# stanfordnlp/mac-network

Measured on AMD Instinct MI355X. Metric: questions/sec fwd+bwd (B=64,d=512,p=12,KB=14x14x1024) at 1/2/4/8 MI355X, higher is better.
Workload: dtype f32 (3xfp16-split emulation); 1 GPU

## Files before the change

mac-network_amd/csrc/macx_chain_h2.hip.h:

```cpp
#pragma once
#include <hip/hip_ext.h>
#include "macx_chain_api.hip.h"

namespace macx {


template <int CTRL>
__device__ __forceinline__ float dpp_mov_f(float v) {
  return __builtin_bit_cast(float, __builtin_amdgcn_update_dpp(0, __builtin_bit_cast(int, v), CTRL, 0xF, 0xF, false));
}
__device__ __forceinline__ float row16_sum(float v) {
  v += dpp_mov_f<0x128>(v);
  v += dpp_mov_f<0x124>(v);
  v += dpp_mov_f<0x122>(v);
  v += dpp_mov_f<0x121>(v);
  return v;
}

__device__ __forceinline__ float row8_sum(float v) {
  v += dpp_mov_f<0x141>(v);
  v += dpp_mov_f<0x1B>(v);
  v += dpp_mov_f<0xB1>(v);
  return v;
}

__device__ __forceinline__ float chain_tanh(float x) {
  const float a = fabsf(x), x2 = x * x;
  float r = 62.0f / 2835.0f;
  r = fmaf(r, x2, -17.0f / 315.0f);
  r = fmaf(r, x2, 2.0f / 15.0f);
  r = fmaf(r, x2, -1.0f / 3.0f);
  r = fmaf(r, x2, 1.0f);
  r *= x;
  const float e = __expf(2.0f * fminf(a, 20.0f));
  const float t = 1.0f - 2.0f * __frcp_rn(e + 1.0f);
  return a < 0.3f ? r : copysignf(t, x);
}
__device__ __forceinline__ float chain_act(int act, float x) {
  if (act == ACT_ELU) return x > 0.0f ? x : __expf(x) - 1.0f;
  if (act == ACT_TANH) return chain_tanh(x);
  return act_apply(act, x);
}

template <int D_, int R_ = 64>
struct ChainGeo {
  static constexpr int D = D_, R = R_, KG = D / 8, CB = D / 128, KS = D / 32;
  static constexpr int TM = 16;
  static constexpr int NWC = D >= 512 ? 8 : 4;
  static constexpr int NWR = 8 / NWC;
  static constexpr int CW = D / NWC;
  static constexpr int RPW = R / NWR;
  static constexpr int RT = RPW / TM;
  static constexpr int CT = CW / 16;
  static constexpr int NRG = R / 16;
  static constexpr int WPG = 8 / NRG;
  static constexpr int IT = KG / (4 * WPG);
  static constexpr int SB = R / 8;
  static_assert(R == 64 || ((R == 32 || R == 16) && NWR == 1), "short tiles: every wave holds all rows (d = 512)");
  static constexpr size_t P_BYTES = (size_t)4 * R * D;
  static constexpr int QS = 5;
  static constexpr int BITS_LD = KG + 4;
  static constexpr size_t LDS = P_BYTES + (size_t)R * (8 + 8 + 1 + 1) * 4 + (size_t)(2 + 1 + QS) * D * 4 + (size_t)R * BITS_LD;
  static_assert((R * BITS_LD) % 16 == 0, "LDS carve-outs stay 16-byte aligned");
  static_assert(D % 128 == 0 && D >= 128 && D <= 512, "one workgroup holds 64 rows x D as H2 planes in LDS");
};

template <int D_, int R_ = 64>
struct ChainCtx {
  using G = ChainGeo<D_, R_>;
// ... 264 lines not shown
  __device__ __forceinline__ float colred_sum(float v) const {
    return row16_sum(v);
  }
  __device__ __forceinline__ bool row_writer() const { return ah == 0; }
  __device__ __forceinline__ bool col_writer() const { return ar == 0; }

  __device__ __forceinline__ void rowmax(const f32x4 (&acc)[RT][CT]) const {
#pragma unroll
    for (int t = 0; t < RT; ++t) {
      float m = 0.f;
#pragma unroll
      for (int c = 0; c < CT; ++c)
#pragma unroll
        for (int q = 0; q < 4; ++q) m = fmaxf(m, fabsf(acc[t][c][q]));
      m = rowred_max(m);
      if (row_writer()) sMax[wave * R + arow(t)] = m;
    }
  }
  __device__ __forceinline__ void emit(const f32x4 (&acc)[RT][CT], bool to_p, const H2View& out) const {
    const size_t Rp = out.Rp();
    const size_t opb = out.plane_bytes();
#pragma unroll
    for (int t = 0; t < RT; ++t) {
      const int row = arow(t);
      const float s = h2_pow2(row_exponent_epi(row));
      const bool st = out.base && row < nvalid;
#pragma unroll
      for (int c = 0; c < CT; ++c) {
        const f32x4 xv = acc[t][c] * s;
        u32x2 hi, lo;
        hi[0] = pk_f16(xv[0], xv[1]);
        hi[1] = pk_f16(xv[2], xv[3]);
        const f32x2_t b0 = unpk_f16(hi[0]), b1 = unpk_f16(hi[1]);
        lo[0] = pk_f16(xv[0] - b0[0], xv[1] - b0[1]);
        lo[1] = pk_f16(xv[2] - b1[0], xv[3] - b1[1]);
        const int kg = akg(c);
        const int half = ahalf();
        if (to_p) {
          char* d = P + ((size_t)kg * R + row) * 16 + half;
          *reinterpret_cast<u32x2*>(d) = hi;
          *reinterpret_cast<u32x2*>(d + (size_t)KG * R * 16) = lo;
        }
        if (st) {
          char* g = out.base + ((size_t)kg * Rp + grow0 + row) * 16 + half;
          *reinterpret_cast<u32x2*>(g) = hi;
          *reinterpret_cast<u32x2*>(g + opb) = lo;
        }
      }
    }
  }
  __device__ __forceinline__ void colsum(const f32x4 (&acc)[RT][CT], float* part) const {
#pragma unroll
    for (int c = 0; c < CT; ++c) {
#pragma unroll
      for (int q = 0; q < 4; ++q) {
        float s = acc[0][c][q];
#pragma unroll
        for (int t = 1; t < RT; ++t) s += acc[t][c][q];
        s = colred_sum(s);
        if (col_writer()) {
          const int col = acol(c) + q;
          if (NWR == 1) part[col] = s;
          else sCol[wr * D + col] = s;
        }
      }
    }
  }
  __device__ __forceinline__ void colsum_finish(float* part) const {
    if (NWR == 2)
      for (int c = tid; c < D; c += 512) part[c] = sCol[c] + sCol[D + c];
  }
};


template <int D_, int KV = 0, int R_ = 64>
__global__ __launch_bounds__(512) void chain_fwd_kernel(const ChainFwdP p) {
  using C = ChainCtx<D_, R_>;
  constexpr int D = C::D, R = C::R, KG = C::KG, CT = C::CT, RT = C::RT, IT = C::IT;
  extern __shared__ __attribute__((aligned(16))) char lds[];
  C x;
  x.init(lds, p.M, p.N);
  const int M = p.M;

  auto stage0 = [&](uint32_t k1, uint32_t k2, uint8_t* bits1, uint8_t* bytes2, const H2View& KBd) __attribute__((always_inline)) {
    float v[IT][8];
    float m = 0.f;
    const bool drop1 = p.thr1 < (1u << 24), drop2 = p.thr2 < (1u << 24);
    const uint32_t key1 = run_key(k1, p.word), key2 = run_key(k2, p.word);
    const size_t Rp2 = (size_t)M + H2_PAD_ROWS;
#pragma unroll
    for (int j = 0; j < IT; ++j) {
      const int kg = x.ckg(j);
      const float* src = p.kb + min(x.cgrow, (size_t)M - 1) * D + kg * 8;
      const f32x4 a0 = *reinterpret_cast<const f32x4*>(src), a1 = *reinterpret_cast<const f32x4*>(src + 4);
#pragma unroll
      for (int q = 0; q < 4; ++q) { v[j][q] = x.cvalid ? a0[q] : 0.f; v[j][4 + q] = x.cvalid ? a1[q] : 0.f; }
    }
#pragma unroll
    for (int j = 0; j < IT; ++j) {
      const int kg = x.ckg(j);
      const uint32_t e0 = p.first + (uint32_t)(x.cgrow * (size_t)p.dlog + kg * 8);
      if (drop1) {
        uint32_t byte = 0;
#pragma unroll
        for (int q = 0; q < 8; q += 2) byte |= keep_pair(e0 + q, key1, p.thr1) << q;
#pragma unroll
        for (int q = 0; q < 8; ++q) v[j][q] = ((byte >> q) & 1u) ? v[j][q] * p.inv1 : 0.f;
        if (bits1 && x.cvalid) bits1[x.cgrow * KG + kg] = (uint8_t)byte;
      }
      if (drop2) {
        uint32_t byte = 0;
#pragma unroll
        for (int q = 0; q < 8; q += 2) byte |= keep_pair(e0 + q, key2, p.thr2) << q;
        x.sBits[x.crow * C::G::BITS_LD + kg] = (uint8_t)byte;
        if (bytes2 && x.cvalid) bytes2[(size_t)kg * Rp2 + x.cgrow] = (uint8_t)byte;
      }
#pragma unroll
      for (int q = 0; q < 8; ++q) m = fmaxf(m, fabsf(v[j][q]));
    }
    x.convert_finish(v, m, x.sE, KBd);
  };
  if constexpr (D == 512) {
#ifdef MACX_FILL_PROF
#define MACX_STAMP(cond, k) do { if ((cond) && p.pre.step == 5 && p.pre.fail && x.tid == 0) p.pre.fail[-31 + (k)] = (uint32_t)__builtin_readcyclecounter(); } while (0)
#else
#define MACX_STAMP(cond, k) do { } while (0)
#endif
    if ((int)blockIdx.x < p.pre.nfill) {
      const int f = blockIdx.x, nf = p.pre.nfill;
      MACX_STAMP(f == 0, 0);
      float (*red)[16][20] = reinterpret_cast<float (*)[16][20]>(lds);
      const int half = x.tid >> 8, tl = x.tid & 255;
      auto signal = [&](uint32_t* c0, uint32_t* c1) __attribute__((always_inline)) {
        asm volatile("s_waitcnt vmcnt(0)" ::: "memory");
        __syncthreads();
        if (x.tid == 0 && c0) signal_counter(c0);
        if (x.tid == 64 && c1) signal_counter(c1);
      };
      static_assert(C::G::P_BYTES >= sizeof(float) * 16 * 16 * 20, "the fillers' linear tiles stay inside P: sPart is free");
      uint32_t* sGave = reinterpret_cast<uint32_t*>(x.sPart);
      auto wait_tiles = [&](uint32_t* ca, uint32_t* cb, uint32_t v) __attribute__((always_inline)) {
        if (x.tid == 0) {
          bool ok = wait_counter<4>(ca, v, HANDOFF_BUDGET, p.pre.fail, p.pre.status, p.pre.step, HANDOFF_WRITE);
          if (ok && cb != ca) ok = wait_counter<4>(cb, v, HANDOFF_BUDGET, p.pre.fail, p.pre.status, p.pre.step, HANDOFF_WRITE);
          *sGave = ok ? 0u : 1u;
        }
        __syncthreads();
        return __builtin_amdgcn_readfirstlane(*sGave) != 0u;
      };
      const bool tail = p.pre.wlin.n_out != 0;
      if (tail) {
        const LinP& wl = p.pre.wlin;
        const int ntx = wl.n_out / 32, nun = ntx * ((wl.rows + 15) / 16);
#pragma unroll 1
        for (int u0 = 2 * f; u0 < nun; u0 += 2 * nf) {
          const int ua = u0, ub = min(u0 + 1, nun - 1), bya = ua / ntx, byb = ub / ntx;
          const int u = half ? ub : ua;
          small_linear_tile<1, false, true, false, 2>(wl, u % ntx, u / ntx, 0, red + 8 * half, tl, u0 + half < nun);
          signal(p.pre.gflag + bya, u0 + 1 < nun ? p.pre.gflag + byb : nullptr);
        }
      }
      MACX_STAMP(f == 0, 1);
      if (p.pre.ylin.n_out) {
        const LinP& yl = p.pre.ylin;
        const int ntx = yl.n_out / 32, nunits = ntx * ((yl.rows + 15) / 16);
        const uint32_t wtiles = (uint32_t)(p.pre.wlin.n_out / 32);
#pragma unroll 1
        for (int u0 = 2 * f; u0 < nunits; u0 += 2 * nf) {
          const int ua = u0, ub = min(u0 + 1, nunits - 1), bya = ua / ntx, byb = ub / ntx;
          const bool gave = tail && wait_tiles(p.pre.gflag + bya, p.pre.gflag + byb, wtiles);
          const int u = half ? ub : ua;
          small_linear_tile<1, false, true, true, 2>(yl, u % ntx, u / ntx, 0, red + 8 * half, tl, u0 + half < nunits, gave);
          __syncthreads();
        }
        signal(p.pre.yflag, nullptr);
      }
      MACX_STAMP(f == 0, 2);
      if (p.pre.KBd.base) {
        const int ntile = (M + R - 1) / R;
#pragma unroll 1
        for (int t = f; t < ntile; t += p.pre.nfill) {
          x.set_tile((size_t)t);
          stage0(p.pre.key1, p.pre.key2, p.pre.bits1, p.pre.bytes2, p.pre.KBd);
        }
      }
      MACX_STAMP(f == 0, 3);
      return;
    }
    x.set_tile((size_t)blockIdx.x - p.pre.nfill);
    MACX_STAMP((int)blockIdx.x == p.pre.nfill, 8);
  }
  if (p.mode == 0) {
    stage0(p.key1, p.key2, p.bits1, p.bytes2, p.KBd);
  } else if (p.mode == 2) {
    if (p.thr2 < (1u << 24)) {
      const size_t Rp2 = (size_t)M + H2_PAD_ROWS;
      const int r = x.tid & 63, k0 = x.tid >> 6;
      const size_t gr = min(x.grow0 + r, (size_t)M - 1);
      if (r < R) {
#pragma unroll
        for (int j = 0; j < KG / 8; ++j) x.sBits[r * C::G::BITS_LD + k0 + 8 * j] = p.bytes2[(size_t)(k0 + 8 * j) * Rp2 + gr];
      }
    }
    x.load_tile(p.KBd, x.sE);
  } else {
    x.load_tile(p.X, x.sE);
  }
  if (p.dbg & 1) return;

  f32x4 acc[RT][CT];
  auto bias_act = [&](auto act_c, const int* eTab, int eW, const float* bias) __attribute__((always_inline)) {
    constexpr int ACT = decltype(act_c)::value;
#pragma unroll
    for (int c = 0; c < CT; ++c) {
      const f32x4 bv = *reinterpret_cast<const f32x4*>(bias + x.acol(c));
#pragma unroll
      for (int t = 0; t < RT; ++t) {
        const float s = h2_unscale(eTab[x.arow(t)], eW);
#pragma unroll
        for (int q = 0; q < 4; ++q) acc[t][c][q] = chain_act(ACT, fmaf(acc[t][c][q], s, bv[q]));
      }
    }
  };
  auto bias_act_any = [&](int act, const int* eTab, int eW, const float* bias) __attribute__((always_inline)) {
    switch (act) {
      case ACT_TANH: bias_act(std::integral_constant<int, ACT_TANH>{}, eTab, eW, bias); break;
      case ACT_SIGMOID: bias_act(std::integral_constant<int, ACT_SIGMOID>{}, eTab, eW, bias); break;
      case ACT_ELU: bias_act(std::integral_constant<int, ACT_ELU>{}, eTab, eW, bias); break;
      case ACT_RELU: bias_act(std::integral_constant<int, ACT_RELU>{}, eTab, eW, bias); break;
      default: bias_act(std::integral_constant<int, ACT_NON>{}, eTab, eW, bias); break;
    }
  };

  if (p.mode != 1) {
    x.zero_acc(acc);
    x.template kloop<KV>(acc, p.Wx.planes);
    bias_act(std::integral_constant<int, ACT_NON>{}, x.sE, *p.Wx.exp, p.bx);
    x.rowmax(acc);
    __syncthreads();
    x.emit(acc, true, p.X);
    x.publish_rows(x.sE, C::PASS_EPI, p.X);
    __syncthreads();
  }
  if (p.dbg & 2) return;

  x.zero_acc(acc);
  x.template kloop<KV>(acc, p.W1b.planes);
  constexpr bool YCOH = D == 512;
  if constexpr (YCOH) {
    MACX_STAMP((int)blockIdx.x == p.pre.nfill, 9);
    if (p.pre.ylin.n_out && x.tid == 0)
      *reinterpret_cast<uint32_t*>(x.sPart) =
          wait_counter<8>(p.pre.yflag, (uint32_t)p.pre.nfill, HANDOFF_BUDGET, p.pre.fail, p.pre.status, p.pre.step, HANDOFF_Y) ? 0u : 1u;
  }
  if constexpr (YCOH) MACX_STAMP((int)blockIdx.x == p.pre.nfill, 10);
  __syncthreads();
  bool ygave = false;
  if constexpr (YCOH) {
    if (p.pre.ylin.n_out) ygave = __builtin_amdgcn_readfirstlane(*reinterpret_cast<const uint32_t*>(x.sPart)) != 0u;
  }
  {
    float v[IT][8];
    float m = 0.f;
    const float inv = h2_pow2(-x.sE[x.crow]);
    const float* yq = p.y + x.qrow(x.cgrow) * D;
    auto ldy = [&](const float* q) __attribute__((always_inline)) {
      if constexpr (YCOH) {
        const uint64_t* q8 = reinterpret_cast<const uint64_t*>(q);
        const uint64_t lo = __hip_atomic_load(q8, __ATOMIC_RELAXED, __HIP_MEMORY_SCOPE_AGENT);
        const uint64_t hi = __hip_atomic_load(q8 + 1, __ATOMIC_RELAXED, __HIP_MEMORY_SCOPE_AGENT);
        return f32x4{__uint_as_float((uint32_t)lo), __uint_as_float((uint32_t)(lo >> 32)), __uint_as_float((uint32_t)hi),
                     __uint_as_float((uint32_t)(hi >> 32))};
      } else {
        return *reinterpret_cast<const f32x4*>(q);
      }
    };
#pragma unroll
    for (int j = 0; j < IT; ++j) {
      const int kg = x.ckg(j);
      const char* s = x.P + ((size_t)kg * R + x.crow) * 16;
      const u32x4 hi = *reinterpret_cast<const u32x4*>(s), lo = *reinterpret_cast<const u32x4*>(s + (size_t)KG * R * 16);
      float xv[8];
      h2_join8(hi, lo, inv, xv);
      const f32x4 y0 = ldy(yq + kg * 8), y1 = ldy(yq + kg * 8 + 4);
#pragma unroll
      for (int q = 0; q < 8; ++q) {
        v[j][q] = xv[q] * (q < 4 ? y0[q & 3] : y1[q & 3]);
        m = fmaxf(m, fabsf(v[j][q]));
      }
    }
    if (ygave) {
#pragma unroll
      for (int j = 0; j < IT; ++j)
#pragma unroll
        for (int q = 0; q < 8; ++q) v[j][q] = handoff_poison();
    }
    x.convert_finish(v, m, x.sE2, H2View{nullptr, M, D});
  }
  {
    const int de = *p.W1a.exp - *p.W1b.exp;
#pragma unroll
    for (int t = 0; t < RT; ++t) {
      const int k = x.sE2[x.arow(t)] - x.sE[x.arow(t)] + de;
#pragma unroll
      for (int c = 0; c < CT; ++c)
#pragma unroll
        for (int q = 0; q < 4; ++q) acc[t][c][q] = ldexpf(acc[t][c][q], k);
    }
  }
  x.template kloop<KV>(acc, p.W1a.planes);
  bias_act_any(p.act1, x.sE2, *p.W1a.exp, p.b1);
  x.rowmax(acc);
  __syncthreads();
  x.emit(acc, true, p.H1);
  x.publish_rows(x.sE, C::PASS_EPI, p.H1);
  __syncthreads();
  if (p.dbg & 4) return;

  x.zero_acc(acc);
  x.template kloop<KV>(acc, p.W2.planes);
  bias_act(std::integral_constant<int, ACT_NON>{}, x.sE, *p.W2.exp, p.b2);
  x.rowmax(acc);
  {
    const bool drop2 = p.thr2 < (1u << 24);
    auto logit_pass = [&](auto act_c) __attribute__((always_inline)) {
      constexpr int ACT = decltype(act_c)::value;
#pragma unroll
      for (int t = 0; t < RT; ++t) {
        const size_t gr = min(x.grow0 + x.arow(t), (size_t)M - 1);
        const float* cq = p.c + (size_t)((uint32_t)gr / (uint32_t)p.N) * D;
        float part = 0.f;
#pragma unroll
        for (int c = 0; c < CT; ++c) {
          const int col = x.acol(c);
          const f32x4 cv = *reinterpret_cast<const f32x4*>(cq + col);
          const f32x4 wv = *reinterpret_cast<const f32x4*>(p.wk + col);
          const uint32_t kb = drop2 ? (uint32_t)x.sBits[x.arow(t) * C::G::BITS_LD + (col >> 3)] >> (col & 4) : 0xFu;
#pragma unroll
          for (int q = 0; q < 4; ++q) {
            float g = chain_act(ACT, acc[t][c][q] * cv[q]);
            if (drop2) g = ((kb >> q) & 1u) ? g * p.inv2 : 0.f;
            part = fmaf(g, wv[q], part);
          }
        }
        part = x.rowred_sum(part);
        if (x.row_writer()) x.sPart[x.wave * R + x.arow(t)] = part;
      }
    };
    switch (p.act2) {
      case ACT_TANH: logit_pass(std::integral_constant<int, ACT_TANH>{}); break;
      case ACT_SIGMOID: logit_pass(std::integral_constant<int, ACT_SIGMOID>{}); break;
      case ACT_ELU: logit_pass(std::integral_constant<int, ACT_ELU>{}); break;
      case ACT_RELU: logit_pass(std::integral_constant<int, ACT_RELU>{}); break;
      default: logit_pass(std::integral_constant<int, ACT_NON>{}); break;
    }
  }
  __syncthreads();
  x.emit(acc, false, p.I2);
  x.publish_rows(x.sE2, C::PASS_EPI, p.I2);
  if constexpr (D == 512) MACX_STAMP((int)blockIdx.x == p.pre.nfill, 11);
  if (x.tid < x.nvalid) {
    const int w0 = (x.tid / C::RPW) * C::NWC;
    float s = x.sPart[w0 * R + x.tid];
#pragma unroll
    for (int w = 1; w < C::NWC; ++w) s += x.sPart[(w0 + w) * R + x.tid];
    p.logits[x.grow0 + x.tid] = ygave ? handoff_poison() : s;
  }
}

template <int D_, int KV = 0, int R_ = 64>
inline hipError_t chain_fwd_launch_t(const ChainFwdP& p, hipStream_t st, hipEvent_t e0, hipEvent_t e1) {
  auto kern = chain_fwd_kernel<D_, KV, R_>;
  constexpr size_t lds = ChainGeo<D_, R_>::LDS;
  hipError_t e = lds_attr_once(reinterpret_cast<const void*>(kern), lds);
  if (e != hipSuccess) return e;
  const int grid = (p.M + R_ - 1) / R_ + (D_ == 512 ? p.pre.nfill : 0);
  if (e0 && e1) hipExtLaunchKernelGGL(kern, dim3(grid), dim3(512), lds, st, e0, e1, 0, p);
  else hipLaunchKernelGGL(kern, dim3(grid), dim3(512), lds, st, p);
  return hipGetLastError();
}


#ifdef MACX_CHAIN_FWD_TU
hipError_t chain_fwd_launch(const ChainFwdP& p, hipStream_t st, hipEvent_t e0, hipEvent_t e1) {
  switch (p.d / 128) {
    case 1: return chain_fwd_launch_t<128>(p, st, e0, e1);
    case 2: return chain_fwd_launch_t<256>(p, st, e0, e1);
    case 3: return chain_fwd_launch_t<384>(p, st, e0, e1);
    case 4:
      switch (chain_tile_rows(p.d, (size_t)p.M)) {
        case 16: return chain_fwd_launch_t<512, 0, 16>(p, st, e0, e1);
        case 32: return chain_fwd_launch_t<512, 0, 32>(p, st, e0, e1);
        default: break;
      }
#ifdef MACX_PROFILE_VARIANTS
      switch (p.dbg >> 3) {
        case 1: return chain_fwd_launch_t<512, 1>(p, st, e0, e1);
        case 2: return chain_fwd_launch_t<512, 2>(p, st, e0, e1);
        case 3: return chain_fwd_launch_t<512, 3>(p, st, e0, e1);
        default: break;
      }
#endif
      return chain_kv() == 0 ? chain_fwd_launch_t<512, 0>(p, st, e0, e1) : chain_fwd_launch_t<512, CHAIN_KV_DEFAULT>(p, st, e0, e1);
    default: return hipErrorInvalidValue;
  }
}
#endif




struct DkbJob { int s, t; bool write, valid; };

template <int KV, class C, class NEXT>
__device__ __forceinline__ void dkb_run(C& x, const ChainDkbP& q, DkbJob job, NEXT next) {
  constexpr int D = C::D, R = C::R, KG = C::KG, CB = C::CB, CT = C::CT, RT = C::RT;
  constexpr int NS = 2 * KG * R / 512;
  static_assert(R == 64 && D == 512 && CT == 4 && RT == 4, "dKB jobs: d = 512, 64-row tiles");
  const size_t Rp = (size_t)x.M + H2_PAD_ROWS;
  u32x4 pf[NS];
// ... 85 lines not shown
          for (int e = 0; e < 4; ++e) {
            const float m = ((nib >> e) & 1u) ? acc[t][c][e] * sc[t] * q.inv_keep : 0.f;
            o[e] = fmaf(a[t], dv[e], m) + (write ? 0.f : old[t][c][e]);
          }
          if (row < x.nvalid) *reinterpret_cast<f32x4*>(q.out + ((size_t)x.grow0 + row) * D + x.colbase + 16 * c + 4 * ah) = o;
        }
      }
    }
    MACX_DSTAMP();
    if (!nj.valid) break;
    job = nj;
    __syncthreads();
  }
}

template <int KV, class C>
__device__ __forceinline__ void dkb_fill(C& x, const ChainDkbP& q, int f) {
  const int ntile = (x.M + C::R - 1) / C::R;
  const int s = q.step;
  const int w0 = q.nskip ? dkb_win0(s, q.nskip, ntile) : 0;
  auto job_of = [&](int j) {
    DkbJob r;
    const int u = f + q.nfill * j;
    r.valid = j < q.njobs && u < ntile - q.nskip;
    r.s = s;
    r.t = u < w0 ? u : u + q.nskip;
    r.write = true;
    for (int s2 = s + 1; s2 < q.p; ++s2) r.write = r.write && q.nskip && dkb_skipped(s2, r.t, q.nskip, ntile);
    return r;
  };
  int j = 0;
  dkb_run<KV>(x, q, job_of(0), [&](const DkbJob&) { return job_of(++j); });
}

template <int D_, int KV>
__global__ __launch_bounds__(512) void chain_dkb_rest_kernel(const ChainDkbP q, int M, int N) {
  using C = ChainCtx<D_, 64>;
  extern __shared__ __attribute__((aligned(16))) char lds[];
  C x;
  x.init(lds, M, N);
  const int ntile = gridDim.x, t = blockIdx.x;
  bool touched = false;
  for (int s = 1; s < q.p; ++s) touched = touched || !(q.nskip && dkb_skipped(s, t, q.nskip, ntile));
  auto below = [&](int s0, bool wr) {
    DkbJob r;
    int s = s0;
    while (s > 0 && !(q.nskip && dkb_skipped(s, t, q.nskip, ntile))) --s;
    r.s = s; r.t = t; r.write = wr; r.valid = s >= 0;
    return r;
  };
  dkb_run<KV>(x, q, below(q.p - 1, !touched), [&](const DkbJob& cur) { return cur.s > 0 ? below(cur.s - 1, false) : DkbJob{0, 0, false, false}; });
}

template <int D_, int KV = 0, int A2 = -1, int R_ = 64>
__global__ __launch_bounds__(512) void chain_bwd_kernel(const ChainBwdP p) {
  using C = ChainCtx<D_, R_>;
  constexpr int D = C::D, R = C::R, KG = C::KG, CB = C::CB, CT = C::CT, RT = C::RT, IT = C::IT;
  extern __shared__ __attribute__((aligned(16))) char lds[];
  C x;
  x.init(lds, p.M, p.N);
  const int M = p.M;
  if constexpr (D == 512 && R == 64) {
    const int ntile = (M + R - 1) / R;
    if ((int)blockIdx.x >= ntile) {
      dkb_fill<KV>(x, p.dkb, (int)blockIdx.x - ntile);
      return;
    }
  }
#ifdef MACX_FILL_PROF
#define MACX_BSTAMP(k) do { if (p.dkb.prof && p.dkb.step == 5 && blockIdx.x == 0 && x.tid == 0) p.dkb.prof[PROF_BWD_OFF + (k)] = (uint32_t)__builtin_readcyclecounter(); } while (0)
#else
#define MACX_BSTAMP(k) do { } while (0)
#endif
  MACX_BSTAMP(0);

  {
    const int q0 = (int)((uint32_t)x.grow0 / (uint32_t)p.N), q1 = (int)(((uint32_t)x.grow0 + x.nvalid - 1) / (uint32_t)p.N);
    const int nq = q1 - q0 + 1;
    float* sRed = x.sPart;
    float* sDot = x.sPart + 64;
    for (int i = x.tid; i < D; i += 512) x.sW[i] = p.wk[i];
    for (int i = x.tid; i < nq * D; i += 512) x.sC[i] = p.c[(size_t)q0 * D + i];
    const int r8 = x.lane & 7, kq = x.lane >> 3;
    const bool active = x.wave < KG / 8;
    const int kg = active ? 8 * x.wave + kq : 0;
    const size_t Rp = p.I2.Rp();
    const size_t ipb = p.I2.plane_bytes();
    const size_t tile = blockIdx.x;
    const bool sums = p.dc_part != nullptr;
    const uint8_t* bytes_src = p.bytes2 ? p.bytes2 : reinterpret_cast<const uint8_t*>(p.I2.base);
    const uint32_t bits_or = p.bytes2 ? 0u : 0xFFu;
    float mx[8] = {0.f, 0.f, 0.f, 0.f, 0.f, 0.f, 0.f, 0.f};
    u32x4 raw[8][2];
    uint32_t bits[8];
    float dlr[8], inv[8];
    int seg[8];
    const char* src0 = p.I2.base + ((size_t)kg * Rp + x.grow0 + r8) * 16;
    const uint8_t* b0 = bytes_src + (size_t)kg * Rp + x.grow0 + r8;
    const int8_t* e0 = p.I2.exps() + (x.grow0 + r8) * CB + (kg >> 4);
    const uint32_t g0 = (uint32_t)x.grow0 + r8, last = (uint32_t)M - 1, un = (uint32_t)p.N;
    const uint32_t qb1 = (uint32_t)(q0 + 1) * un, qb2 = qb1 + un;
    constexpr bool EARLY = (KG / 8) >= 8 && C::SB >= 3;
    int eraw[3];
    float a_r[3], d_r[3];
    auto fetch_a = [&](auto sb_c) __attribute__((always_inline)) {
      constexpr int sb = decltype(sb_c)::value;
      raw[sb][0] = *reinterpret_cast<const u32x4*>(src0 + sb * 128);
      raw[sb][1] = *reinterpret_cast<const u32x4*>(src0 + ipb + sb * 128);
      bits[sb] = (uint32_t)b0[sb * 8];
      eraw[sb] = (int)e0[sb * 8 * CB];
      const uint32_t gr = min(g0 + 8 * sb, last);
      a_r[sb] = p.att[gr];
      d_r[sb] = p.da[gr];
    };
    if constexpr (EARLY) {
      fetch_a(std::integral_constant<int, 0>{});
      fetch_a(std::integral_constant<int, 1>{});
      fetch_a(std::integral_constant<int, 2>{});
    }
    {
      float part[C::G::QS];
#pragma unroll
      for (int k = 0; k < C::G::QS; ++k) {
        part[k] = 0.f;
        if (k < nq) {
          const float* aq = p.att + (size_t)(q0 + k) * p.N;
          const float* dq = p.da + (size_t)(q0 + k) * p.N;
          for (int n = x.tid; n < p.N; n += 512) part[k] += aq[n] * dq[n];
        }
      }
#pragma unroll
      for (int k = 0; k < C::G::QS; ++k)
        if (k < nq) {
          const float t = wave_sum(part[k]);
          if (x.lane == 0) sRed[k * 8 + x.wave] = t;
        }
      __syncthreads();
      if (x.tid < nq) {
        float t = 0.f;
#pragma unroll
        for (int w = 0; w < 8; ++w) t += sRed[x.tid * 8 + w];
        sDot[x.tid] = t;
      }
      __syncthreads();
    }
    auto fetch = [&](auto sb_c) __attribute__((always_inline)) {
      constexpr int sb = decltype(sb_c)::value;
      raw[sb][0] = *reinterpret_cast<const u32x4*>(src0 + sb * 128);
      raw[sb][1] = *reinterpret_cast<const u32x4*>(src0 + ipb + sb * 128);
      bits[sb] = (uint32_t)b0[sb * 8];
      inv[sb] = h2_pow2(-(int)e0[sb * 8 * CB]);
      const uint32_t gr = min(g0 + 8 * sb, last);
      seg[sb] = nq <= 3 ? (int)(gr >= qb1) + (int)(gr >= qb2) : (int)(gr / un) - q0;
      const float dl_row = p.att[gr] * (p.da[gr] - sDot[seg[sb]]);
      dlr[sb] = 8 * sb + r8 < x.nvalid ? dl_row : 0.f;
    };
    auto fetch_b = [&](auto sb_c) __attribute__((always_inline)) {
      constexpr int sb = decltype(sb_c)::value;
      if constexpr (sb < 3) {
        inv[sb] = h2_pow2(-eraw[sb]);
        const uint32_t gr = min(g0 + 8 * sb, last);
        seg[sb] = nq <= 3 ? (int)(gr >= qb1) + (int)(gr >= qb2) : (int)(gr / un) - q0;
        dlr[sb] = 8 * sb + r8 < x.nvalid ? a_r[sb] * (d_r[sb] - sDot[seg[sb]]) : 0.f;
      }
    };
    float a_dw[8], a_db[8], a_dc[3][8];
#pragma unroll
    for (int e = 0; e < 8; ++e) a_dw[e] = a_db[e] = a_dc[0][e] = a_dc[1][e] = a_dc[2][e] = 0.f;
    const f32x4 w0 = *reinterpret_cast<const f32x4*>(x.sW + kg * 8), w1 = *reinterpret_cast<const f32x4*>(x.sW + kg * 8 + 4);
    auto block = [&](auto act_c, auto sb_c) __attribute__((always_inline)) {
      constexpr int ACTC = decltype(act_c)::value;
      const int ACT = ACTC >= 0 ? ACTC : p.act2;
      constexpr int sb = decltype(sb_c)::value;
      const float* cq = x.sC + (size_t)seg[sb] * D + kg * 8;
      const f32x4 c0 = *reinterpret_cast<const f32x4*>(cq), c1 = *reinterpret_cast<const f32x4*>(cq + 4);
      float i2[8];
      h2_join8(raw[sb][0], raw[sb][1], inv[sb], i2);
      const bool rv = 8 * sb + r8 < x.nvalid;
      float o[8];
      float m = 0.f;
#pragma unroll
      for (int e = 0; e < 8; ++e) {
        i2[e] = rv ? i2[e] : 0.f;
        const float cv = e < 4 ? c0[e & 3] : c1[e & 3], wv = e < 4 ? w0[e & 3] : w1[e & 3];
        const float g = chain_act(ACT, i2[e] * cv);
        const float f = (((bits[sb] | bits_or) >> e) & 1u) ? p.inv2 : 0.f;
        const float dz = (dlr[sb] * wv) * f * act_grad_from_out(ACT, g);
        const float ov = dz * cv;
        o[e] = ov;
        m = fmaxf(m, fabsf(ov));
        a_dw[e] = fmaf(dlr[sb], g * f, a_dw[e]);
        a_db[e] += ov;
        const float t = dz * i2[e];
        a_dc[0][e] += seg[sb] == 0 ? t : 0.f;
        a_dc[1][e] += seg[sb] == 1 ? t : 0.f;
        a_dc[2][e] += seg[sb] == 2 ? t : 0.f;
      }
      mx[sb] = m;
      x.blk_park(kg, 8 * sb + r8, o);
    };
    auto pass = [&](auto act_c) __attribute__((always_inline)) {
      constexpr int SBc = C::SB;
      constexpr int PFD = 3;
      if constexpr (EARLY) {
        fetch_b(std::integral_constant<int, 0>{});
        fetch_b(std::integral_constant<int, 1>{});
        fetch_b(std::integral_constant<int, 2>{});
      } else {
        fetch(std::integral_constant<int, 0>{});
        if constexpr (SBc > 1) fetch(std::integral_constant<int, 1>{});
        if constexpr (SBc > 2 && PFD > 2) fetch(std::integral_constant<int, 2>{});
      }
      __builtin_amdgcn_sched_barrier(0);
      auto step = [&](auto sb_c) __attribute__((always_inline)) {
        constexpr int sb = decltype(sb_c)::value;
        if constexpr (sb < SBc) {
          if constexpr (sb + PFD < SBc) fetch(std::integral_constant<int, sb + PFD>{});
          block(act_c, sb_c);
          __builtin_amdgcn_sched_barrier(0);
        }
      };
      step(std::integral_constant<int, 0>{}); step(std::integral_constant<int, 1>{}); step(std::integral_constant<int, 2>{});
      step(std::integral_constant<int, 3>{}); step(std::integral_constant<int, 4>{}); step(std::integral_constant<int, 5>{});
      step(std::integral_constant<int, 6>{}); step(std::integral_constant<int, 7>{});
    };
    if (active) pass(std::integral_constant<int, A2>{});
    if (sums && active) {
      float* dw = p.dwk_part + tile * D + kg * 8;
      float* db = p.db2_part + tile * D + kg * 8;
      float* dc = p.dc_part + tile * 3 * D + kg * 8;
#pragma unroll
      for (int e = 0; e < 8; ++e) {
        a_dw[e] = row8_sum(a_dw[e]);
        a_db[e] = row8_sum(a_db[e]);
#pragma unroll
        for (int k = 0; k < 3; ++k)
          if (k < nq) a_dc[k][e] = row8_sum(a_dc[k][e]);
      }
      if (r8 == 0) {
        *reinterpret_cast<f32x4*>(dw) = f32x4{a_dw[0], a_dw[1], a_dw[2], a_dw[3]};
        *reinterpret_cast<f32x4*>(dw + 4) = f32x4{a_dw[4], a_dw[5], a_dw[6], a_dw[7]};
        *reinterpret_cast<f32x4*>(db) = f32x4{a_db[0], a_db[1], a_db[2], a_db[3]};
        *reinterpret_cast<f32x4*>(db + 4) = f32x4{a_db[4], a_db[5], a_db[6], a_db[7]};
#pragma unroll
        for (int k = 0; k < 3; ++k)
          if (k < nq) {
            *reinterpret_cast<f32x4*>(dc + k * D) = f32x4{a_dc[k][0], a_dc[k][1], a_dc[k][2], a_dc[k][3]};
            *reinterpret_cast<f32x4*>(dc + k * D + 4) = f32x4{a_dc[k][4], a_dc[k][5], a_dc[k][6], a_dc[k][7]};
          }
      }
    }
    if (sums && x.tid < 64) {
      const uint32_t gr = min((uint32_t)x.grow0 + x.tid, (uint32_t)M - 1);
      const int sg = (int)(gr / (uint32_t)p.N) - q0;
      const float dl = x.tid < x.nvalid ? p.att[gr] * (p.da[gr] - sDot[sg]) : 0.f;
#pragma unroll
      for (int k = 0; k < 3; ++k) {
        const float t = wave_sum(sg == k ? dl : 0.f);
        if (x.tid == 0) p.dls_part[tile * 3 + k] = t;
      }
    }
    x.convert_finish_blk(mx, p.dI2, x.sE);
  }
  MACX_BSTAMP(1);
  if (p.dbg & 1) return;

  f32x4 acc[RT][CT];
  const size_t tile = blockIdx.x;
  x.zero_acc(acc);
  x.template kloop<KV>(acc, p.W2T.planes);
  MACX_BSTAMP(2);
  {
    const int eW = *p.W2T.exp;
    const size_t Rp = p.H1.Rp();
    const size_t hpb = p.H1.plane_bytes();
    auto pass = [&](auto act_c) __attribute__((always_inline)) {
      constexpr int ACT = decltype(act_c)::value;
#pragma unroll
      for (int t = 0; t < RT; ++t) {
        const size_t gr = min(x.grow0 + x.arow(t), (size_t)M - 1);
        const float s = h2_unscale(x.sE[x.arow(t)], eW);
        const int8_t* ex = p.H1.exps() + gr * CB;
#pragma unroll
        for (int c = 0; c < CT; ++c) {
          const int kg = x.akg(c);
          const char* src = p.H1.base + ((size_t)kg * Rp + gr) * 16 + x.ahalf();
          const u32x2 hh = *reinterpret_cast<const u32x2*>(src), hl = *reinterpret_cast<const u32x2*>(src + hpb);
          float h[4];
          h2_join4(hh, hl, h2_pow2(-(int)ex[kg >> 4]), h);
#pragma unroll
          for (int q = 0; q < 4; ++q) acc[t][c][q] = acc[t][c][q] * s * act_grad_from_out(ACT, h[q]);
        }
      }
    };
    switch (p.act1) {
      case ACT_TANH: pass(std::integral_constant<int, ACT_TANH>{}); break;
      case ACT_SIGMOID: pass(std::integral_constant<int, ACT_SIGMOID>{}); break;
      case ACT_ELU: pass(std::integral_constant<int, ACT_ELU>{}); break;
      case ACT_RELU: pass(std::integral_constant<int, ACT_RELU>{}); break;
      default: pass(std::integral_constant<int, ACT_NON>{}); break;
    }
  }
  x.colsum(acc, p.db1_part + tile * D);
  x.rowmax(acc);
  __syncthreads();
  x.emit(acc, true, p.dI1);
  x.publish_rows(x.sE, C::PASS_EPI, p.dI1);
  x.colsum_finish(p.db1_part + tile * D);
  __syncthreads();
  MACX_BSTAMP(3);
  if (p.dbg & 2) return;

  x.zero_acc(acc);
  x.template kloop<KV>(acc, p.W1aT.planes);
  MACX_BSTAMP(4);
  if (p.dy_part) {
    const int q0 = (int)((uint32_t)x.grow0 / (uint32_t)p.N), q1 = (int)(((uint32_t)x.grow0 + x.nvalid - 1) / (uint32_t)p.N);
    const int nq = q1 - q0 + 1;
    const uint32_t qb1 = (uint32_t)(q0 + 1) * (uint32_t)p.N, qb2 = qb1 + (uint32_t)p.N;
    const int eW = *p.W1aT.exp;
    const size_t Rp = p.X.Rp();
    const size_t xpb = p.X.plane_bytes();
    float sr[RT];
    int sg[RT];
    size_t gr[RT];
#pragma unroll
    for (int t = 0; t < RT; ++t) {
      gr[t] = min(x.grow0 + x.arow(t), (size_t)M - 1);
      sg[t] = (int)((uint32_t)gr[t] >= qb1) + (int)((uint32_t)gr[t] >= qb2);
      sr[t] = h2_unscale(x.sE[x.arow(t)], eW);
    }
    float* stage = x.sW;
#pragma unroll
    for (int c = 0; c < CT; ++c) {
      const int kg = x.akg(c);
      float xv[RT][4];
#pragma unroll
      for (int t = 0; t < RT; ++t) {
        const char* src = p.X.base + ((size_t)kg * Rp + gr[t]) * 16 + x.ahalf();
        const u32x2 hh = *reinterpret_cast<const u32x2*>(src), hl = *reinterpret_cast<const u32x2*>(src + xpb);
        h2_join4(hh, hl, h2_pow2(-(int)p.X.exps()[gr[t] * CB + (kg >> 4)]), xv[t]);
      }
#pragma unroll
      for (int q = 0; q < 4; ++q) {
        float s3[3] = {0.f, 0.f, 0.f};
#pragma unroll
        for (int t = 0; t < RT; ++t) {
          const float v = x.arow(t) < x.nvalid ? acc[t][c][q] * sr[t] * xv[t][q] : 0.f;
          s3[0] += sg[t] == 0 ? v : 0.f;
          s3[1] += sg[t] == 1 ? v : 0.f;
          s3[2] += sg[t] == 2 ? v : 0.f;
        }
        const int col = x.acol(c) + q;
#pragma unroll
        for (int k = 0; k < 3; ++k)
          if (k < nq) {
            const float sum = x.colred_sum(s3[k]);
            if (x.col_writer()) {
              if (C::NWR == 1) p.dy_part[(tile * 3 + k) * D + col] = sum;
              else stage[(x.wr * 3 + k) * D + col] = sum;
            }
          }
      }
    }
  }
  {
    const int de = *p.W1bT.exp - *p.W1aT.exp;
#pragma unroll
    for (int t = 0; t < RT; ++t) {
      const float* yq = p.y + x.qrow(x.grow0 + x.arow(t)) * D;
#pragma unroll
      for (int c = 0; c < CT; ++c) {
        const f32x4 yv = *reinterpret_cast<const f32x4*>(yq + x.acol(c));
#pragma unroll
        for (int q = 0; q < 4; ++q) acc[t][c][q] = ldexpf(acc[t][c][q] * yv[q], de);
      }
    }
  }
  MACX_BSTAMP(5);
  x.template kloop<KV>(acc, p.W1bT.planes);
  MACX_BSTAMP(6);
  {
    const int eW = *p.W1bT.exp;
#pragma unroll
    for (int t = 0; t < RT; ++t) {
      const float s = h2_unscale(x.sE[x.arow(t)], eW);
#pragma unroll
      for (int c = 0; c < CT; ++c) acc[t][c] *= s;
    }
  }
  x.colsum(acc, p.dbx_part + tile * D);
  x.rowmax(acc);
  __syncthreads();
  x.emit(acc, false, p.dX);
  x.publish_rows(x.sE2, C::PASS_EPI, p.dX);
  x.colsum_finish(p.dbx_part + tile * D);
  MACX_BSTAMP(7);
  if (C::NWR == 2 && p.dy_part) {
    const int nq = (int)(((uint32_t)x.grow0 + x.nvalid - 1) / (uint32_t)p.N) - (int)((uint32_t)x.grow0 / (uint32_t)p.N) + 1;
    for (int i = x.tid; i < nq * D; i += 512) p.dy_part[tile * 3 * D + i] = x.sW[i] + x.sW[3 * D + i];
  }
}

template <int D_, int KV, int A2, int R_ = 64>
inline hipError_t chain_bwd_launch_a(const ChainBwdP& p, hipStream_t st) {
  auto kern = chain_bwd_kernel<D_, KV, A2, R_>;
  constexpr size_t lds = ChainGeo<D_, R_>::LDS;
  hipError_t e = lds_attr_once(reinterpret_cast<const void*>(kern), lds);
  if (e != hipSuccess) return e;
  const int nfill = (D_ == 512 && R_ == 64 && p.dkb.njobs > 0) ? p.dkb.nfill : 0;
  hipLaunchKernelGGL(kern, dim3((p.M + R_ - 1) / R_ + nfill), dim3(512), lds, st, p);
  return hipGetLastError();
}

template <int D_, int KV = 0, int R_ = 64>
inline hipError_t chain_bwd_launch_t(const ChainBwdP& p, hipStream_t st) {
  switch (p.act2) {
    case ACT_ELU: return chain_bwd_launch_a<D_, KV, ACT_ELU, R_>(p, st);
    case ACT_RELU: return chain_bwd_launch_a<D_, KV, ACT_RELU, R_>(p, st);
    case ACT_TANH: return chain_bwd_launch_a<D_, KV, ACT_TANH, R_>(p, st);
    case ACT_SIGMOID: return chain_bwd_launch_a<D_, KV, ACT_SIGMOID, R_>(p, st);
    default: return chain_bwd_launch_a<D_, KV, ACT_NON, R_>(p, st);
  }
}

#ifdef MACX_CHAIN_BWD_TU
hipError_t chain_dkb_rest_launch(const ChainDkbP& q, int M, int N, int d, hipStream_t st) {
  if (d != 512 || chain_tile_rows(d, (size_t)M) != 64) return hipErrorInvalidValue;
  auto kern = chain_dkb_rest_kernel<512, CHAIN_KV_DEFAULT>;
  constexpr size_t lds = ChainGeo<512, 64>::LDS;
  hipError_t e = lds_attr_once(reinterpret_cast<const void*>(kern), lds);
  if (e != hipSuccess) return e;
  hipLaunchKernelGGL(kern, dim3((M + 63) / 64), dim3(512), lds, st, q, M, N);
  return hipGetLastError();
}

hipError_t chain_bwd_launch(const ChainBwdP& p, hipStream_t st) {
  switch (p.d / 128) {
    case 1: return chain_bwd_launch_t<128>(p, st);
    case 2: return chain_bwd_launch_t<256>(p, st);
    case 3: return chain_bwd_launch_t<384>(p, st);
    case 4:
      switch (chain_tile_rows(p.d, (size_t)p.M)) {
        case 16: return chain_bwd_launch_t<512, 0, 16>(p, st);
        case 32: return chain_bwd_launch_t<512, 0, 32>(p, st);
        default: break;
      }
      if (p.act2 != ACT_ELU) return chain_bwd_launch_t<512, CHAIN_KV_DEFAULT>(p, st);
#ifdef MACX_PROFILE_VARIANTS
      switch (p.dbg >> 3) {
        case 1: return chain_bwd_launch_a<512, 1, ACT_ELU>(p, st);
        case 3: return chain_bwd_launch_a<512, 3, ACT_ELU>(p, st);
        default: break;
      }
#endif
      return chain_kv() == 0 ? chain_bwd_launch_a<512, 0, ACT_ELU>(p, st) : chain_bwd_launch_a<512, CHAIN_KV_DEFAULT, ACT_ELU>(p, st);
    default: return hipErrorInvalidValue;
  }
}
#endif


}
```

mac-network_amd/csrc/macx_common.hip.h:

```cpp
#pragma once
#include <hip/hip_runtime.h>
#include <stdint.h>
#include <mutex>
#include <map>
#include <set>
#include <utility>
#include "../../include/macx.h"

typedef float f32x4 __attribute__((ext_vector_type(4)));
typedef float f32x16 __attribute__((ext_vector_type(16)));

namespace macx {

inline hipError_t lds_attr_once(const void* fn, size_t bytes) {
  static std::mutex mu;
  static std::set<std::pair<const void*, int>> done;
  int dev = 0;
  hipError_t e = hipGetDevice(&dev);
  if (e != hipSuccess) return e;
  std::lock_guard<std::mutex> lock(mu);
  if (done.count({fn, dev})) return hipSuccess;
  e = hipFuncSetAttribute(fn, hipFuncAttributeMaxDynamicSharedMemorySize, (int)bytes);
  if (e == hipSuccess) done.insert({fn, dev});
  return e;
// ... 63 lines not shown
};

struct DropSpec {
  uint32_t key;
  uint32_t thr24;
  float inv_keep;
  const uint32_t* word;
};

__device__ __forceinline__ uint32_t run_key(uint32_t key, const uint32_t* word) { return word ? key ^ *word : key; }
__device__ __forceinline__ uint32_t run_key(const DropSpec& d) { return run_key(d.key, d.word); }

__device__ __forceinline__ DropSpec drop_resolve(DropSpec d) { d.key = run_key(d); d.word = nullptr; return d; }
__device__ __forceinline__ float drop_apply(float v, uint32_t idx, const DropSpec& d) {
  return keep_bit(idx, d.key, d.thr24) ? v * d.inv_keep : 0.0f;
}

enum : int { ACT_NON = 0, ACT_TANH = 1, ACT_SIGMOID = 2, ACT_ELU = 3, ACT_RELU = 4 };

__device__ __forceinline__ float elu_f(float x) {
  const float e = __expf(x) - 1.0f;
  float r = 1.0f / 5040.0f;
  r = fmaf(r, x, 1.0f / 720.0f);
  r = fmaf(r, x, 1.0f / 120.0f);
  r = fmaf(r, x, 1.0f / 24.0f);
  r = fmaf(r, x, 1.0f / 6.0f);
  r = fmaf(r, x, 0.5f);
  r = fmaf(r, x, 1.0f);
  r *= x;
  return x > 0.0f ? x : (x > -0.35f ? r : e);
}
__device__ __forceinline__ float elu_grad_from_out(float h) { return h > 0.0f ? 1.0f : h + 1.0f; }
__device__ __forceinline__ float elu_grad_from_in(float x) { return x > 0.0f ? 1.0f : expf(x); }

__device__ __forceinline__ float act_apply(int act, float x) {
  switch (act) {
    case ACT_TANH: return tanhf(x);
    case ACT_SIGMOID: return 1.0f / (1.0f + expf(-x));
    case ACT_ELU: return elu_f(x);
    case ACT_RELU: return fmaxf(x, 0.0f);
    default: return x;
  }
}
__device__ __forceinline__ float act_grad_from_out(int act, float o) {
  switch (act) {
    case ACT_TANH: return 1.0f - o * o;
    case ACT_SIGMOID: return o * (1.0f - o);
    case ACT_ELU: return elu_grad_from_out(o);
    case ACT_RELU: return o > 0.0f ? 1.0f : 0.0f;
    default: return 1.0f;
  }
}

__device__ __forceinline__ float wave_sum(float v) {
#pragma unroll
  for (int o = 32; o > 0; o >>= 1) v += __shfl_xor(v, o, 64);
  return v;
}
__device__ __forceinline__ float wave_max(float v) {
#pragma unroll
  for (int o = 32; o > 0; o >>= 1) v = fmaxf(v, __shfl_xor(v, o, 64));
  return v;
}
__device__ __forceinline__ float half_sum(float v) {
#pragma unroll
  for (int o = 16; o > 0; o >>= 1) v += __shfl_xor(v, o, 64);
  return v;
}

}
```

Before: 18560 questions/s.

## Batch DPP column reductions, use bitmask selects, add two-question backward specialization

Column sums now batch several independent values through each DPP row16 reduction step, which should expose more instruction-level parallelism than reducing one value at a time. Conditional selects for validity and dropout masks are replaced by AND-with-lane-mask bit tricks so the compiler emits VALU ANDs instead of compare/cndmask pairs. A TWO template specialization of the backward kernel, used for 64-row tiles when N is at least 64 and the activation is not linear, tracks only two question segments, cutting accumulator registers and select work. Assembly stage marker macros are added for inspection. Both the 3-segment staging buffer and the TWO path assume a tile spans at most two questions, and the masking relies on compiler-opaque asm barriers.

```diff
diff --git a/mac-network_amd/csrc/macx_chain_h2.hip.h b/mac-network_amd/csrc/macx_chain_h2.hip.h
--- a/mac-network_amd/csrc/macx_chain_h2.hip.h
+++ b/mac-network_amd/csrc/macx_chain_h2.hip.h
@@ -15,6 +15,21 @@
   v += dpp_mov_f<0x122>(v);
   v += dpp_mov_f<0x121>(v);
   return v;
+}
+template <int CTRL, int NV>
+__device__ __forceinline__ void row16_step_n(float (&v)[NV]) {
+  float t[NV];
+#pragma unroll
+  for (int i = 0; i < NV; ++i) t[i] = dpp_mov_f<CTRL>(v[i]);
+#pragma unroll
+  for (int i = 0; i < NV; ++i) v[i] += t[i];
+}
+template <int NV>
+__device__ __forceinline__ void row16_sum_n(float (&v)[NV]) {
+  row16_step_n<0x128>(v);
+  row16_step_n<0x124>(v);
+  row16_step_n<0x122>(v);
+  row16_step_n<0x121>(v);
 }
 
 __device__ __forceinline__ float row8_sum(float v) {
@@ -385,17 +400,18 @@
   __device__ __forceinline__ void colsum(const f32x4 (&acc)[RT][CT], float* part) const {
 #pragma unroll
     for (int c = 0; c < CT; ++c) {
+      float s[4];
 #pragma unroll
       for (int q = 0; q < 4; ++q) {
-        float s = acc[0][c][q];
-#pragma unroll
-        for (int t = 1; t < RT; ++t) s += acc[t][c][q];
-        s = colred_sum(s);
-        if (col_writer()) {
-          const int col = acol(c) + q;
-          if (NWR == 1) part[col] = s;
-          else sCol[wr * D + col] = s;
-        }
+        s[q] = acc[0][c][q];
+#pragma unroll
+        for (int t = 1; t < RT; ++t) s[q] += acc[t][c][q];
+      }
+      row16_sum_n(s);
+      if (col_writer()) {
+        float* dst = NWR == 1 ? part : sCol + wr * D;
+#pragma unroll
+        for (int q = 0; q < 4; ++q) dst[acol(c) + q] = s[q];
       }
     }
   }
@@ -421,13 +437,14 @@
     const bool drop1 = p.thr1 < (1u << 24), drop2 = p.thr2 < (1u << 24);
     const uint32_t key1 = run_key(k1, p.word), key2 = run_key(k2, p.word);
     const size_t Rp2 = (size_t)M + H2_PAD_ROWS;
+    const uint32_t cvm = lane_mask(x.cvalid);
 #pragma unroll
     for (int j = 0; j < IT; ++j) {
       const int kg = x.ckg(j);
       const float* src = p.kb + min(x.cgrow, (size_t)M - 1) * D + kg * 8;
       const f32x4 a0 = *reinterpret_cast<const f32x4*>(src), a1 = *reinterpret_cast<const f32x4*>(src + 4);
 #pragma unroll
-      for (int q = 0; q < 4; ++q) { v[j][q] = x.cvalid ? a0[q] : 0.f; v[j][4 + q] = x.cvalid ? a1[q] : 0.f; }
+      for (int q = 0; q < 4; ++q) { v[j][q] = mask_f(a0[q], cvm); v[j][4 + q] = mask_f(a1[q], cvm); }
     }
 #pragma unroll
     for (int j = 0; j < IT; ++j) {
@@ -438,7 +455,7 @@
 #pragma unroll
         for (int q = 0; q < 8; q += 2) byte |= keep_pair(e0 + q, key1, p.thr1) << q;
 #pragma unroll
-        for (int q = 0; q < 8; ++q) v[j][q] = ((byte >> q) & 1u) ? v[j][q] * p.inv1 : 0.f;
+        for (int q = 0; q < 8; ++q) v[j][q] = mask_f(v[j][q] * p.inv1, bit_mask(byte, q));
         if (bits1 && x.cvalid) bits1[x.cgrow * KG + kg] = (uint8_t)byte;
       }
       if (drop2) {
@@ -540,6 +557,7 @@
     x.load_tile(p.X, x.sE);
   }
   if (p.dbg & 1) return;
+  MACX_MARK("fwd 0");
 
   f32x4 acc[RT][CT];
   auto bias_act = [&](auto act_c, const int* eTab, int eW, const float* bias) __attribute__((always_inline)) {
@@ -568,6 +586,7 @@
   if (p.mode != 1) {
     x.zero_acc(acc);
     x.template kloop<KV>(acc, p.Wx.planes);
+    MACX_MARK("fwd 1");
     bias_act(std::integral_constant<int, ACT_NON>{}, x.sE, *p.Wx.exp, p.bx);
     x.rowmax(acc);
     __syncthreads();
@@ -576,9 +595,11 @@
     __syncthreads();
   }
   if (p.dbg & 2) return;
+  MACX_MARK("fwd 2");
 
   x.zero_acc(acc);
   x.template kloop<KV>(acc, p.W1b.planes);
+  MACX_MARK("fwd 3");
   constexpr bool YCOH = D == 512;
   if constexpr (YCOH) {
     MACX_STAMP((int)blockIdx.x == p.pre.nfill, 9);
@@ -641,7 +662,9 @@
         for (int q = 0; q < 4; ++q) acc[t][c][q] = ldexpf(acc[t][c][q], k);
     }
   }
+  MACX_MARK("fwd 4");
   x.template kloop<KV>(acc, p.W1a.planes);
+  MACX_MARK("fwd 5");
   bias_act_any(p.act1, x.sE2, *p.W1a.exp, p.b1);
   x.rowmax(acc);
   __syncthreads();
@@ -649,13 +672,16 @@
   x.publish_rows(x.sE, C::PASS_EPI, p.H1);
   __syncthreads();
   if (p.dbg & 4) return;
+  MACX_MARK("fwd 6");
 
   x.zero_acc(acc);
   x.template kloop<KV>(acc, p.W2.planes);
+  MACX_MARK("fwd 7");
   bias_act(std::integral_constant<int, ACT_NON>{}, x.sE, *p.W2.exp, p.b2);
   x.rowmax(acc);
   {
     const bool drop2 = p.thr2 < (1u << 24);
+    const float inv2 = drop2 ? p.inv2 : 1.0f;
     auto logit_pass = [&](auto act_c) __attribute__((always_inline)) {
       constexpr int ACT = decltype(act_c)::value;
 #pragma unroll
@@ -672,7 +698,7 @@
 #pragma unroll
           for (int q = 0; q < 4; ++q) {
             float g = chain_act(ACT, acc[t][c][q] * cv[q]);
-            if (drop2) g = ((kb >> q) & 1u) ? g * p.inv2 : 0.f;
+            g = mask_f(g * inv2, bit_mask(kb, q));
             part = fmaf(g, wv[q], part);
           }
         }
@@ -699,6 +725,7 @@
     for (int w = 1; w < C::NWC; ++w) s += x.sPart[(w0 + w) * R + x.tid];
     p.logits[x.grow0 + x.tid] = ygave ? handoff_poison() : s;
   }
+  MACX_MARK("fwd 8");
 }
 
 template <int D_, int KV = 0, int R_ = 64>
@@ -890,8 +917,9 @@
   dkb_run<KV>(x, q, below(q.p - 1, !touched), [&](const DkbJob& cur) { return cur.s > 0 ? below(cur.s - 1, false) : DkbJob{0, 0, false, false}; });
 }
 
-template <int D_, int KV = 0, int A2 = -1, int R_ = 64>
+template <int D_, int KV = 0, int A2 = -1, int R_ = 64, bool TWO = false>
 __global__ __launch_bounds__(512) void chain_bwd_kernel(const ChainBwdP p) {
+  static_assert(!TWO || R_ == 64, "two-question tiles: the 64-row tile only (the short tiles serve small N and B)");
   using C = ChainCtx<D_, R_>;
   constexpr int D = C::D, R = C::R, KG = C::KG, CB = C::CB, CT = C::CT, RT = C::RT, IT = C::IT;
   extern __shared__ __attribute__((aligned(16))) char lds[];
@@ -906,9 +934,9 @@
     }
   }
 #ifdef MACX_FILL_PROF
-#define MACX_BSTAMP(k) do { if (p.dkb.prof && p.dkb.step == 5 && blockIdx.x == 0 && x.tid == 0) p.dkb.prof[PROF_BWD_OFF + (k)] = (uint32_t)__builtin_readcyclecounter(); } while (0)
+#define MACX_BSTAMP(k) do { MACX_MARK("bwd " #k); if (p.dkb.prof && p.dkb.step == 5 && blockIdx.x == 0 && x.tid == 0) p.dkb.prof[PROF_BWD_OFF + (k)] = (uint32_t)__builtin_readcyclecounter(); } while (0)
 #else
-#define MACX_BSTAMP(k) do { } while (0)
+#define MACX_BSTAMP(k) MACX_MARK("bwd " #k)
 #endif
   MACX_BSTAMP(0);
 
@@ -1002,10 +1030,16 @@
         dlr[sb] = 8 * sb + r8 < x.nvalid ? a_r[sb] * (d_r[sb] - sDot[seg[sb]]) : 0.f;
       }
     };
-    float a_dw[8], a_db[8], a_dc[3][8];
-#pragma unroll
-    for (int e = 0; e < 8; ++e) a_dw[e] = a_db[e] = a_dc[0][e] = a_dc[1][e] = a_dc[2][e] = 0.f;
+    constexpr int NSEG = TWO ? 2 : 3;
+    float a_dw[8], a_db[8], a_dc[NSEG][8];
+#pragma unroll
+    for (int e = 0; e < 8; ++e) {
+      a_dw[e] = a_db[e] = 0.f;
+#pragma unroll
+      for (int k = 0; k < NSEG; ++k) a_dc[k][e] = 0.f;
+    }
     const f32x4 w0 = *reinterpret_cast<const f32x4*>(x.sW + kg * 8), w1 = *reinterpret_cast<const f32x4*>(x.sW + kg * 8 + 4);
+    const uint32_t inv2b = __float_as_uint(p.inv2);
     auto block = [&](auto act_c, auto sb_c) __attribute__((always_inline)) {
       constexpr int ACTC = decltype(act_c)::value;
       const int ACT = ACTC >= 0 ? ACTC : p.act2;
@@ -1015,14 +1049,17 @@
       float i2[8];
       h2_join8(raw[sb][0], raw[sb][1], inv[sb], i2);
       const bool rv = 8 * sb + r8 < x.nvalid;
+      const uint32_t rvm = lane_mask(rv);
+      const uint32_t kbits = bits[sb] | bits_or;
+      const uint32_t second = lane_mask(seg[sb] != 0);
       float o[8];
       float m = 0.f;
 #pragma unroll
       for (int e = 0; e < 8; ++e) {
-        i2[e] = rv ? i2[e] : 0.f;
+        i2[e] = TWO ? mask_f(i2[e], rvm) : (rv ? i2[e] : 0.f);
         const float cv = e < 4 ? c0[e & 3] : c1[e & 3], wv = e < 4 ? w0[e & 3] : w1[e & 3];
         const float g = chain_act(ACT, i2[e] * cv);
-        const float f = (((bits[sb] | bits_or) >> e) & 1u) ? p.inv2 : 0.f;
+        const float f = TWO ? __uint_as_float(bit_mask(kbits, e) & inv2b) : (((kbits >> e) & 1u) ? p.inv2 : 0.f);
         const float dz = (dlr[sb] * wv) * f * act_grad_from_out(ACT, g);
         const float ov = dz * cv;
         o[e] = ov;
@@ -1030,9 +1067,14 @@
         a_dw[e] = fmaf(dlr[sb], g * f, a_dw[e]);
         a_db[e] += ov;
         const float t = dz * i2[e];
-        a_dc[0][e] += seg[sb] == 0 ? t : 0.f;
-        a_dc[1][e] += seg[sb] == 1 ? t : 0.f;
-        a_dc[2][e] += seg[sb] == 2 ? t : 0.f;
+        if constexpr (TWO) {
+          const float t1 = mask_f(t, second);
+          a_dc[0][e] += __uint_as_float(__float_as_uint(t) ^ __float_as_uint(t1));
+          a_dc[1][e] += t1;
+        } else {
+#pragma unroll
+          for (int k = 0; k < NSEG; ++k) a_dc[k][e] += seg[sb] == k ? t : 0.f;
+        }
       }
       mx[sb] = m;
       x.blk_park(kg, 8 * sb + r8, o);
@@ -1072,7 +1114,7 @@
         a_dw[e] = row8_sum(a_dw[e]);
         a_db[e] = row8_sum(a_db[e]);
 #pragma unroll
-        for (int k = 0; k < 3; ++k)
+        for (int k = 0; k < NSEG; ++k)
           if (k < nq) a_dc[k][e] = row8_sum(a_dc[k][e]);
       }
       if (r8 == 0) {
@@ -1081,7 +1123,7 @@
         *reinterpret_cast<f32x4*>(db) = f32x4{a_db[0], a_db[1], a_db[2], a_db[3]};
         *reinterpret_cast<f32x4*>(db + 4) = f32x4{a_db[4], a_db[5], a_db[6], a_db[7]};
 #pragma unroll
-        for (int k = 0; k < 3; ++k)
+        for (int k = 0; k < NSEG; ++k)
           if (k < nq) {
             *reinterpret_cast<f32x4*>(dc + k * D) = f32x4{a_dc[k][0], a_dc[k][1], a_dc[k][2], a_dc[k][3]};
             *reinterpret_cast<f32x4*>(dc + k * D + 4) = f32x4{a_dc[k][4], a_dc[k][5], a_dc[k][6], a_dc[k][7]};
@@ -1169,36 +1211,40 @@
       sr[t] = h2_unscale(x.sE[x.arow(t)], eW);
     }
     float* stage = x.sW;
-#pragma unroll
-    for (int c = 0; c < CT; ++c) {
-      const int kg = x.akg(c);
-      float xv[RT][4];
-#pragma unroll
-      for (int t = 0; t < RT; ++t) {
-        const char* src = p.X.base + ((size_t)kg * Rp + gr[t]) * 16 + x.ahalf();
-        const u32x2 hh = *reinterpret_cast<const u32x2*>(src), hl = *reinterpret_cast<const u32x2*>(src + xpb);
-        h2_join4(hh, hl, h2_pow2(-(int)p.X.exps()[gr[t] * CB + (kg >> 4)]), xv[t]);
-      }
-#pragma unroll
-      for (int q = 0; q < 4; ++q) {
-        float s3[3] = {0.f, 0.f, 0.f};
+    {
+      constexpr int NSEG = TWO ? 2 : 3;
+#pragma unroll
+      for (int c = 0; c < CT; ++c) {
+        const int kg = x.akg(c);
+        float xv[RT][4];
 #pragma unroll
         for (int t = 0; t < RT; ++t) {
-          const float v = x.arow(t) < x.nvalid ? acc[t][c][q] * sr[t] * xv[t][q] : 0.f;
-          s3[0] += sg[t] == 0 ? v : 0.f;
-          s3[1] += sg[t] == 1 ? v : 0.f;
-          s3[2] += sg[t] == 2 ? v : 0.f;
-        }
-        const int col = x.acol(c) + q;
-#pragma unroll
-        for (int k = 0; k < 3; ++k)
-          if (k < nq) {
-            const float sum = x.colred_sum(s3[k]);
-            if (x.col_writer()) {
-              if (C::NWR == 1) p.dy_part[(tile * 3 + k) * D + col] = sum;
-              else stage[(x.wr * 3 + k) * D + col] = sum;
+          const char* src = p.X.base + ((size_t)kg * Rp + gr[t]) * 16 + x.ahalf();
+          const u32x2 hh = *reinterpret_cast<const u32x2*>(src), hl = *reinterpret_cast<const u32x2*>(src + xpb);
+          h2_join4(hh, hl, h2_pow2(-(int)p.X.exps()[gr[t] * CB + (kg >> 4)]), xv[t]);
+        }
+        float s[4 * NSEG];
+#pragma unroll
+        for (int q = 0; q < 4; ++q) {
+#pragma unroll
+          for (int k = 0; k < NSEG; ++k) s[q * NSEG + k] = 0.f;
+#pragma unroll
+          for (int t = 0; t < RT; ++t) {
+            const float v = x.arow(t) < x.nvalid ? acc[t][c][q] * sr[t] * xv[t][q] : 0.f;
+#pragma unroll
+            for (int k = 0; k < NSEG; ++k) s[q * NSEG + k] += sg[t] == k ? v : 0.f;
+          }
+        }
+        row16_sum_n(s);
+        if (x.col_writer()) {
+#pragma unroll
+          for (int k = 0; k < NSEG; ++k)
+            if (k < nq) {
+              float* dst = C::NWR == 1 ? p.dy_part + (tile * 3 + k) * D : stage + (x.wr * 3 + k) * D;
+#pragma unroll
+              for (int q = 0; q < 4; ++q) dst[x.acol(c) + q] = s[q * NSEG + k];
             }
-          }
+        }
       }
     }
   }
@@ -1240,15 +1286,22 @@
   }
 }
 
-template <int D_, int KV, int A2, int R_ = 64>
-inline hipError_t chain_bwd_launch_a(const ChainBwdP& p, hipStream_t st) {
-  auto kern = chain_bwd_kernel<D_, KV, A2, R_>;
+template <int D_, int KV, int A2, int R_, bool TWO>
+inline hipError_t chain_bwd_launch_k(const ChainBwdP& p, hipStream_t st) {
+  auto kern = chain_bwd_kernel<D_, KV, A2, R_, TWO>;
   constexpr size_t lds = ChainGeo<D_, R_>::LDS;
   hipError_t e = lds_attr_once(reinterpret_cast<const void*>(kern), lds);
   if (e != hipSuccess) return e;
   const int nfill = (D_ == 512 && R_ == 64 && p.dkb.njobs > 0) ? p.dkb.nfill : 0;
   hipLaunchKernelGGL(kern, dim3((p.M + R_ - 1) / R_ + nfill), dim3(512), lds, st, p);
   return hipGetLastError();
+}
+template <int D_, int KV, int A2, int R_ = 64>
+inline hipError_t chain_bwd_launch_a(const ChainBwdP& p, hipStream_t st) {
+  if constexpr (R_ == 64 && A2 != ACT_NON) {
+    if (p.N >= R_) return chain_bwd_launch_k<D_, KV, A2, R_, true>(p, st);
+  }
+  return chain_bwd_launch_k<D_, KV, A2, R_, false>(p, st);
 }
 
 template <int D_, int KV = 0, int R_ = 64>
diff --git a/mac-network_amd/csrc/macx_common.hip.h b/mac-network_amd/csrc/macx_common.hip.h
--- a/mac-network_amd/csrc/macx_common.hip.h
+++ b/mac-network_amd/csrc/macx_common.hip.h
@@ -139,6 +139,24 @@
   }
 }
 
+#ifdef MACX_STAGE_MARKS
+#define MACX_MARK(name) asm volatile("; MACX_STAGE " name)
+#else
+#define MACX_MARK(name) do { } while (0)
+#endif
+
+__device__ __forceinline__ uint32_t lane_mask(bool c) {
+  uint32_t m = c ? ~0u : 0u;
+  asm("" : "+v"(m));
+  return m;
+}
+__device__ __forceinline__ float mask_f(float v, uint32_t m) { return __uint_as_float(__float_as_uint(v) & m); }
+__device__ __forceinline__ uint32_t bit_mask(uint32_t bits, int e) {
+  uint32_t m = (uint32_t)__builtin_amdgcn_sbfe((int)bits, (uint32_t)e, 1u);
+  asm("" : "+v"(m));
+  return m;
+}
+
 __device__ __forceinline__ float wave_sum(float v) {
 #pragma unroll
   for (int o = 32; o > 0; o >>= 1) v += __shfl_xor(v, o, 64);
```

Result: faster. 18840 questions/s, median of 6 (+1.5%).
